# ulrikisdahl/MuZero-Breakout

Measured on AMD Instinct MI355X. Metric: env-steps/sec (whole node) at N_envs×N_sims; visit-count match vs CPU ref, higher is better.
Workload: dtype bf16

## Files before the change

### muzero-breakout_amd/csrc/towerp.hip

```cpp
#include "common.h"
#include "tree_dev.h"
#include "elt.h"

namespace {

constexpr int TP_STAGE = 2;

namespace tp {
constexpr int E = 16;
constexpr int P = 20;
constexpr int ROWS = E * P;
constexpr int C = 256;
constexpr int ROWB = C * 2;
constexpr int IMG = ROWS * ROWB;
constexpr int PIX = E * ROWB;
constexpr int NT = 256;
constexpr int CT = 4;
constexpr int TNS = 72;
constexpr int CTB = TNS * 1024;
MZ_DEV int off(int row, int chunk) { return row * ROWB + ((chunk ^ (row & 15)) << 4); }
MZ_DEV uint32_t relu_pk(uint32_t u) {
  uint32_t r;
  asm("v_pk_max_i16 %0, %1, 0" : "=v"(r) : "v"(u));
  return r;
}
}

#ifdef TOWERP_STAMPS
constexpr int PST_N = 192, PST_WG = 256;
__device__ unsigned long long mz_towerp_stamps[PST_WG * 4][PST_N];
MZ_DEV void pstamp(int k, bool real = false) {
  if ((threadIdx.x & 63) == 0 && blockIdx.x < PST_WG && k < PST_N)
    mz_towerp_stamps[blockIdx.x * 4 + (threadIdx.x >> 6)][k] = real ? __builtin_amdgcn_s_memrealtime() : __builtin_amdgcn_s_memtime();
}
#define PSTAMP(k) pstamp(k)
#else
#define PSTAMP(k) \
  do {            \
  } while (0)
#endif

struct TPW {
  __amdgpu_buffer_rsrc_t rs;
  MZ_DEV uint4 ld(int ct, int step, int lane) const {
    return __builtin_bit_cast(uint4, __builtin_amdgcn_raw_buffer_load_b128(rs, lane * 16, ct * tp::CTB + step * 1024, 0));
  }
};
MZ_DEV TPW tpw(const void* pack, int ct0) {
  const uint4* p = reinterpret_cast<const uint4*>(pack) + (size_t)ct0 * tp::TNS * 64;
  return TPW{__builtin_amdgcn_make_buffer_rsrc(const_cast<uint4*>(p), 0, 0x7fffffff, 0x00020000)};
}

MZ_DEV TPW tpw1(const void* pack, int ct0) {
  const uint4* p = reinterpret_cast<const uint4*>(pack) + (size_t)ct0 * 8 * 64;
  return TPW{__builtin_amdgcn_make_buffer_rsrc(const_cast<uint4*>(p), 0, 0x7fffffff, 0x00020000)};
}

MZ_DEV void tp_preload(uint4 (&bq)[2][3][2], const TPW& w, int lane) {
#pragma unroll
  for (int cc = 0; cc < 2; ++cc)
#pragma unroll
    for (int d = 0; d < 3; ++d)
#pragma unroll
      for (int ct = 0; ct < 2; ++ct) bq[cc][d][ct] = w.ld(ct, 24 * d + cc, lane);
}

template <int EL, int DYI>
__device__ __forceinline__ void tp_dy(const uint8_t* __restrict__ lds, int lb, int q, int n, const TPW& cur,
                                      const TPW& nxt, uint4 (&bq)[2][3][2], f32x4 (&acc)[tp::P][2],
                                      typename Elt<EL>::v8 (&fa)[5], typename Elt<EL>::v8 (&fb)[5], int lane) {
  typedef typename Elt<EL>::v8 V8;
  constexpr int DY = DYI - 1;
  constexpr int YLO = DY < 0 ? 0 : DY, YHI = DY > 0 ? 3 : 3 + DY, NY = YHI - YLO + 1;
  constexpr int NYLO = DYI == 0 ? 0 : (DYI == 1 ? 1 : 0);
#pragma unroll 1
  for (int cp = 0; cp < 4; ++cp) {
#pragma unroll
    for (int cc = 0; cc < 2; ++cc) {
      const int c = 2 * cp + cc, s = 8 * DYI + c;
      const bool wrap = cc == 1 && cp == 3;
      const int cn = wrap ? 0 : c + 1;
      const int xc = lb + (((4 * c + q) ^ n) << 4), xn = lb + (((4 * cn + q) ^ n) << 4);
      const int ynext = wrap ? NYLO : YLO;
      int st = s + 2;
      __amdgpu_buffer_rsrc_t rs = cur.rs;
      if (DYI == 2) {
        rs = st >= 24 ? nxt.rs : cur.rs;
        st = st >= 24 ? st - 24 : st;
      }
#pragma unroll
      for (int yi = 0; yi < NY; ++yi) {
        const int yp = YLO + yi;
        const int nb = yi + 1 < NY ? xc + 5 * (yp + 1) * tp::PIX : xn + 5 * ynext * tp::PIX;
        const bool last = yi == NY - 1;
        auto row = [&](const V8(&f)[5], V8(&fn)[5]) {
          V8 w[3][2];
#pragma unroll
          for (int d = 0; d < 3; ++d)
#pragma unroll
            for (int ct = 0; ct < 2; ++ct) w[d][ct] = __builtin_bit_cast(V8, bq[cc][d][ct]);
#pragma unroll
          for (int xp = 0; xp < 5; ++xp)
#pragma unroll
            for (int ct = 0; ct < 2; ++ct)
              acc[(yp - DY) * 5 + xp][ct] = Elt<EL>::mfma(w[1][ct], f[xp], acc[(yp - DY) * 5 + xp][ct]);
#pragma unroll
          for (int xp = 0; xp < 5; ++xp) fn[xp] = *reinterpret_cast<const V8*>(lds + nb + xp * tp::PIX);
#pragma unroll
          for (int xp = 0; xp < 4; ++xp)
#pragma unroll
            for (int ct = 0; ct < 2; ++ct)
              acc[(yp - DY) * 5 + xp + 1][ct] = Elt<EL>::mfma(w[0][ct], f[xp], acc[(yp - DY) * 5 + xp + 1][ct]);
#pragma unroll
          for (int xp = 1; xp < 5; ++xp)
#pragma unroll
            for (int ct = 0; ct < 2; ++ct)
              acc[(yp - DY) * 5 + xp - 1][ct] = Elt<EL>::mfma(w[2][ct], f[xp], acc[(yp - DY) * 5 + xp - 1][ct]);
          if (last) {
#pragma unroll
            for (int ct = 0; ct < 2; ++ct)
#pragma unroll
              for (int d = 0; d < 3; ++d)
                bq[cc][d][ct] = __builtin_bit_cast(
                    uint4, __builtin_amdgcn_raw_buffer_load_b128(rs, lane * 16, ct * tp::CTB + (24 * d + st) * 1024, 0));
          }
          __builtin_amdgcn_sched_group_barrier(0x008, 8, 0);
#pragma unroll
          for (int j = 0; j < 5; ++j) {
            __builtin_amdgcn_sched_group_barrier(0x008, 1, 0);
            __builtin_amdgcn_sched_group_barrier(0x100, 1, 0);
          }
          __builtin_amdgcn_sched_group_barrier(0x008, 13, 0);
          if (last) __builtin_amdgcn_sched_group_barrier(0x020, 6, 0);
          __builtin_amdgcn_sched_barrier(0);
        };
        if (((cc * NY + yi) & 1) == 0)
          row(fa, fb);
        else
          row(fb, fa);
      }
    }
  }
}

struct TPArgs {
  const bf16_t* in;
  long long in_env_stride;
  const int32_t* slot;
  long long in_slot_stride;
  bf16_t* out;
  const bf16_t* wf;
  const float* bias;
  int nblocks;
  int B;
  mzba_tower_ext x;
  TreeArgs tree;
  int tree_on, tree_sim;
  float tree_gamma;
  const float* tree_r;
};

template <int EL, int MODE>
MZ_DEV void tp_init1(f32x4 (&acc)[2], const float4 (&bias)[2], int chb, const uint2 (&res)[2],
                     const float* __restrict__ actb, int act, int A, int q, int p) {
#pragma unroll
  for (int ct = 0; ct < 2; ++ct) {
    const int ch = chb + 16 * ct + 4 * q;
    const float4 b4 = bias[ct];
    f32x4 v = {b4.x, b4.y, b4.z, b4.w};
    if (MODE == 1) {
      const uint2 r = res[ct];
      v[0] += Elt<EL>::lo(r.x); v[1] += Elt<EL>::hi(r.x);
      v[2] += Elt<EL>::lo(r.y); v[3] += Elt<EL>::hi(r.y);
    } else if (MODE == 2) {
      const float4 t = *reinterpret_cast<const float4*>(actb + ((size_t)p * A + act) * tp::C + ch);
      v[0] += t.x; v[1] += t.y; v[2] += t.z; v[3] += t.w;
    }
    acc[ct] = v;
  }
}
template <int EL, int MODE>
MZ_DEV void tp_init(f32x4 (&acc)[tp::P][2], const float4 (&bias)[2], int chb, const uint2 (&res)[tp::P][2],
                    const float* __restrict__ actb, int act, int A, int q) {
#pragma unroll
  for (int p = 0; p < tp::P; ++p) tp_init1<EL, MODE>(acc[p], bias, chb, res[p], actb, act, A, q, p);
}
MZ_DEV void tp_pin(f32x4 (&acc)[tp::P][2]) {
#pragma unroll
  for (int p = 0; p < tp::P; ++p)
#pragma unroll
    for (int ct = 0; ct < 2; ++ct) asm volatile("" : "+a"(acc[p][ct]));
}

MZ_DEV void tp_bias(float4 (&b)[2], const float* __restrict__ bias, int chb, int q) {
#pragma unroll
  for (int ct = 0; ct < 2; ++ct) b[ct] = *reinterpret_cast<const float4*>(bias + chb + 16 * ct + 4 * q);
}

template <int EL>
MZ_DEV void tp_k3(const uint8_t* __restrict__ lds, int lb, int q, int n, const TPW& cur, const TPW& nxt,
                  uint4 (&bq)[2][3][2], typename Elt<EL>::v8 (&fa)[5], typename Elt<EL>::v8 (&fb)[5],
                  f32x4 (&acc)[tp::P][2], int lane) {
  tp_dy<EL, 0>(lds, lb, q, n, cur, nxt, bq, acc, fa, fb, lane);
  tp_dy<EL, 1>(lds, lb, q, n, cur, nxt, bq, acc, fa, fb, lane);
  tp_dy<EL, 2>(lds, lb, q, n, cur, nxt, bq, acc, fa, fb, lane);
}

template <int EL>
MZ_DEV void tp_k1(const uint8_t* __restrict__ lds, int lb, int q, int n, const TPW& w, f32x4 (&acc)[tp::P][2],
                  int lane) {
  typedef typename Elt<EL>::v8 V8;
  uint4 wq[8][2];
#pragma unroll
  for (int c = 0; c < 8; ++c)
#pragma unroll
    for (int ct = 0; ct < 2; ++ct)
      wq[c][ct] = __builtin_bit_cast(uint4, __builtin_amdgcn_raw_buffer_load_b128(w.rs, lane * 16, ct * 8192 + c * 1024, 0));
  V8 fa[5], fb[5];
  auto rd = [&](int k, V8(&f)[5]) {
    const int xc = lb + (((4 * (k >> 2) + q) ^ n) << 4), yp = k & 3;
#pragma unroll
    for (int xp = 0; xp < 5; ++xp) f[xp] = *reinterpret_cast<const V8*>(lds + xc + (5 * yp + xp) * tp::PIX);
  };
  rd(0, fa);
#pragma unroll
  for (int k = 0; k < 32; ++k) {
    auto step = [&](const V8(&f)[5], V8(&fn)[5]) {
      const int c = k >> 2, yp = k & 3;
      if (k + 1 < 32) rd(k + 1, fn);
#pragma unroll
      for (int ct = 0; ct < 2; ++ct)
#pragma unroll
        for (int xp = 0; xp < 5; ++xp)
          acc[5 * yp + xp][ct] = Elt<EL>::mfma(__builtin_bit_cast(V8, wq[c][ct]), f[xp], acc[5 * yp + xp][ct]);
      if (k + 1 < 32) {
#pragma unroll
        for (int j = 0; j < 5; ++j) {
          __builtin_amdgcn_sched_group_barrier(0x008, 1, 0);
          __builtin_amdgcn_sched_group_barrier(0x100, 1, 0);
        }
        __builtin_amdgcn_sched_group_barrier(0x008, 5, 0);
      }
      __builtin_amdgcn_sched_barrier(0);
    };
    if (k & 1)
      step(fb, fa);
    else
      step(fa, fb);
  }
}

template <int EL>
MZ_DEV uint2 tp_pack(const f32x4& a) {
  return make_uint2(tp::relu_pk(Elt<EL>::pack2(a[0], a[1])), tp::relu_pk(Elt<EL>::pack2(a[2], a[3])));
}
MZ_DEV int tp_cofs(int ch, int n) { return n * tp::ROWB + (((ch >> 3) ^ n) << 4) + ((ch & 7) << 1); }

template <int EL>
MZ_DEV void tp_first_frags(const uint8_t* __restrict__ lds, int lb, int q, int n, typename Elt<EL>::v8 (&fa)[5]) {
  const int x0 = lb + ((q ^ n) << 4);
#pragma unroll
  for (int xp = 0; xp < 5; ++xp) fa[xp] = *reinterpret_cast<const typename Elt<EL>::v8*>(lds + x0 + xp * tp::PIX);
}

template <int EL, int MODE, bool SAVE>
__device__ __forceinline__ void tp_conv(uint8_t* __restrict__ lds, const uint4* w, const TPW& wn,
                                        const float* __restrict__ bias, float4 (&bc)[2], const float* __restrict__ nbias,
                                        uint2 (&res)[2][tp::P][2],
                                        const float* __restrict__ actb, int act, int A, uint4 (&bq)[2][3][2], int lane,
                                        int wave, int ci) {
  const int q = lane >> 4, n = lane & 15;
  const int lb = n * tp::ROWB;
  const int ct0 = tp::CT * wave;
  const TPW w0 = tpw(w, ct0), w1 = tpw(w, ct0 + 2);
  PSTAMP(2 + 5 * ci);
  typename Elt<EL>::v8 fa[5], fb[5];
  tp_first_frags<EL>(lds, lb, q, n, fa);
  uint2 out0[tp::P][2];
  f32x4 acc[tp::P][2];
  tp_init<EL, MODE>(acc, bc, 64 * wave, res[0], actb, act, A, q);
  tp_pin(acc);
  float4 b1[2];
  tp_bias(b1, bias, 64 * wave + 32, q);
  tp_k3<EL>(lds, lb, q, n, w0, w1, bq, fa, fb, acc, lane);
  PSTAMP(3 + 5 * ci);
#pragma unroll
  for (int p = 0; p < tp::P; ++p) {
#pragma unroll
    for (int ct = 0; ct < 2; ++ct) out0[p][ct] = tp_pack<EL>(acc[p][ct]);
    tp_init1<EL, MODE>(acc[p], b1, 64 * wave + 32, res[1][p], actb, act, A, q, p);
    __builtin_amdgcn_sched_barrier(0);
  }
  tp_pin(acc);
  tp_bias(bc, nbias, 64 * wave, q);
  tp_k3<EL>(lds, lb, q, n, w1, wn, bq, fa, fb, acc, lane);
  PSTAMP(4 + 5 * ci);
  __syncthreads();
  PSTAMP(5 + 5 * ci);
  int cofs[tp::CT];
#pragma unroll
  for (int ct = 0; ct < tp::CT; ++ct) cofs[ct] = tp_cofs(64 * wave + 16 * ct + 4 * q, n);
#pragma unroll
  for (int p = 0; p < tp::P; ++p) {
#pragma unroll
    for (int ct = 0; ct < tp::CT; ++ct) {
      uint2* ptr = reinterpret_cast<uint2*>(lds + p * tp::PIX + cofs[ct]);
      if (SAVE) res[ct >> 1][p][ct & 1] = *ptr;
      *ptr = ct < 2 ? out0[p][ct] : tp_pack<EL>(acc[p][ct - 2]);
    }
    __builtin_amdgcn_sched_barrier(0);
  }
  __syncthreads();
  PSTAMP(6 + 5 * ci);
}

constexpr int TPH_PART = 0, TPH_LG = 2048, TPH_DEC = 2560, TPH_TAB = 2688;
template <int EL, int NH, int C0, int C1>
MZ_DEV void tp_heads(const TPArgs& a, uint8_t* __restrict__ lds, const int (&hc0)[2], const int (&kind)[2], int env0,
                     int nenv, int tid) {
  constexpr int NU0 = 20 * C0 / 32 / 4, NU1 = NH > 1 ? 20 * C1 / 32 / 4 : 0, NU = NU0 + NU1;
  static_assert(NU <= 40, "head weight batch");
  const int nh = NH;
  const int lane = tid & 63, wave = tid >> 6, q = lane >> 4, el = lane & 15;
  typedef typename Elt<EL>::v8 V8;
  f32x4 hacc[2] = {{0.f, 0.f, 0.f, 0.f}, {0.f, 0.f, 0.f, 0.f}};
  V8 bv[NU];
#pragma unroll
  for (int u = 0; u < NU; ++u) {
    const int hd = u < NU0 ? 0 : 1, K = 20 * (hd ? C1 : C0), s = wave + 4 * (hd ? u - NU0 : u);
    bv[u] = *reinterpret_cast<const V8*>(reinterpret_cast<const bf16_t*>(a.x.lw[hd]) + (size_t)el * K + s * 32 + q * 8);
  }
#pragma unroll
  for (int u = 0; u < NU; ++u) {
    const int hd = u < NU0 ? 0 : 1, C = hd ? C1 : C0, s = wave + 4 * (hd ? u - NU0 : u);
    const int k = s * 32 + q * 8;
    const int pos = k / C, c = hc0[hd] + (k - pos * C);
    const V8 av = *reinterpret_cast<const V8*>(lds + tp::off(pos * tp::E + el, c >> 3));
    hacc[hd] = Elt<EL>::mfma(av, bv[u], hacc[hd]);
  }
  __syncthreads();
  float* sc = reinterpret_cast<float*>(lds);
  float* part = sc + TPH_PART;
  float* lg = sc + TPH_LG;
  float* dec = sc + TPH_DEC;
#pragma unroll
  for (int hd = 0; hd < 2; ++hd)
    if (hd < nh)
#pragma unroll
      for (int i = 0; i < 4; ++i) part[((hd * 4 + wave) * 16 + 4 * q + i) * 16 + el] = hacc[hd][i];
  __syncthreads();
  for (int hd = 0; hd < nh; ++hd) {
    const int e = tid >> 4, o = tid & 15;
    float v = 0.f;
#pragma unroll
    for (int w = 0; w < 4; ++w) v = v + part[((hd * 4 + w) * 16 + e) * 16 + o];
    if (o < a.x.lO[hd]) lg[(hd * 16 + e) * 16 + o] = v + a.x.lb[hd][o];
  }
  __syncthreads();
  if (tid < 16 * nh) {
    const int hd = tid >> 4, e = tid & 15, b = env0 + e;
    if (e < nenv) {
      const int O = a.x.lO[hd];
      float l[16];
      for (int o = 0; o < O; ++o) {
        l[o] = lg[(hd * 16 + e) * 16 + o];
        if (a.x.logits[hd]) a.x.logits[hd][(size_t)b * O + o] = l[o];
      }
      if (kind[hd] == 0) {
        float m = l[0];
        for (int o = 1; o < O; ++o) m = fmaxf(m, l[o]);
        float ex[16], sum = 0.f;
        for (int o = 0; o < O; ++o) { ex[o] = expf(l[o] - m); sum = sum + ex[o]; }
        for (int o = 0; o < O; ++o) {
          const float p = ex[o] / sum;
          a.x.dec[hd][(size_t)b * O + o] = p;
          if (o < 4) dec[(hd * 16 + e) * 4 + o] = p;
        }
      } else {
        const float d = decode_support(l, O, a.x.smin, a.x.smax);
        a.x.dec[hd][b] = d;
        dec[(hd * 16 + e) * 4] = d;
      }
    }
  }
}

template <int EL>
MZ_DEV void tp_scale(const TPArgs& a, const uint8_t* __restrict__ lds, int env0, int nenv, int tid) {
  const int e = tid >> 4, t = tid & 15;
  uint32_t mn2 = 0xffffffffu, mx2 = 0u;
#pragma unroll 8
  for (int u = 0; u < 40; ++u) {
    const int i = u * 16 + t, p = i >> 5, c = i & 31;
    const uint4 v = *reinterpret_cast<const uint4*>(lds + tp::off(p * tp::E + e, c));
    const uint32_t w4[4] = {v.x, v.y, v.z, v.w};
#pragma unroll
    for (int j = 0; j < 4; ++j) {
      asm("v_pk_min_u16 %0, %1, %2" : "=v"(mn2) : "v"(mn2), "v"(w4[j]));
      asm("v_pk_max_u16 %0, %1, %2" : "=v"(mx2) : "v"(mx2), "v"(w4[j]));
    }
  }
  const uint32_t mnh = min(mn2 & 0xffffu, mn2 >> 16), mxh = max(mx2 & 0xffffu, mx2 >> 16);
  float mn = Elt<EL>::lo(mnh), mx = Elt<EL>::lo(mxh);
  for (int o = 8; o > 0; o >>= 1) { mn = fminf(mn, __shfl_xor(mn, o)); mx = fmaxf(mx, __shfl_xor(mx, o)); }
  if (e >= nenv) return;
  const float den = (mx - mn) + 1e-8f;
  const double rden = 1.0 / (double)den;
  auto dv = [&](float x) { return (float)((double)(x - mn) * rden); };
  const int b = env0 + e;
  bf16_t* o1 = a.out ? a.out + (size_t)b * 20 * tp::C : nullptr;
  bf16_t* o2 = a.x.pool ? reinterpret_cast<bf16_t*>(a.x.pool) + (size_t)b * a.x.pool_env_stride +
                              (size_t)a.x.pool_slot * 20 * tp::C
                        : nullptr;
#pragma unroll 4
  for (int u = 0; u < 40; ++u) {
    const int i = u * 16 + t, p = i >> 5, c = i & 31;
    const uint4 v = *reinterpret_cast<const uint4*>(lds + tp::off(p * tp::E + e, c));
    float f[8];
    unpack8<EL>(v, f);
    const uint4 r = make_uint4(pack_bf16x2(dv(f[0]), dv(f[1])), pack_bf16x2(dv(f[2]), dv(f[3])),
                               pack_bf16x2(dv(f[4]), dv(f[5])), pack_bf16x2(dv(f[6]), dv(f[7])));
    if (o1) *reinterpret_cast<uint4*>(o1 + p * tp::C + c * 8) = r;
    if (o2) *reinterpret_cast<uint4*>(o2 + p * tp::C + c * 8) = r;
  }
}

template <int EL>
__global__ __launch_bounds__(tp::NT, 1) void towerp_kernel(TPArgs a) {
  __shared__ __attribute__((aligned(16))) uint8_t lds[tp::IMG];
  const int tid = threadIdx.x, lane = tid & 63;
  const int wave = __builtin_amdgcn_readfirstlane(tid >> 6);
  const int q = lane >> 4, n = lane & 15, lb = n * tp::ROWB;
  const int env0 = blockIdx.x * tp::E;
  const int nenv = min(tp::E, a.B - env0);
  const uint4* wf = reinterpret_cast<const uint4*>(a.wf);
  constexpr size_t WCONV = (size_t)16 * tp::TNS * 64;
  const bool pro = a.x.w0 != nullptr;
  const int ct0 = tp::CT * wave;
  PSTAMP(0);
#ifdef TOWERP_STAMPS
  pstamp(PST_N - 3, true);
#endif
  uint4 bq[2][3][2];
  tp_preload(bq, tpw(pro ? a.x.w0 : a.wf, ct0), lane);
  const int act = pro ? a.x.act[env0 + (n < nenv ? n : 0)] : 0;
  constexpr int SB = 4 / TP_STAGE;
#pragma unroll
  for (int h = 0; h < TP_STAGE; ++h) {
    uint4 v[10 * SB];
#pragma unroll
    for (int bb = 0; bb < SB; ++bb) {
      const int e = 4 * wave + SB * h + bb;
      const bool ok = e < nenv;
      const int b = env0 + (ok ? e : 0);
      const long long eo = (long long)b * a.in_env_stride + (a.slot ? (long long)a.slot[b] * a.in_slot_stride : 0);
#pragma unroll
      for (int u = 0; u < 10; ++u) {
        v[bb * 10 + u] = Elt<EL>::from_bf16(*reinterpret_cast<const uint4*>(a.in + eo + (long long)(u * 64 + lane) * 8));
        if (!ok) v[bb * 10 + u] = make_uint4(0, 0, 0, 0);
      }
    }
#pragma unroll
    for (int bb = 0; bb < SB; ++bb) {
      const int e = 4 * wave + SB * h + bb;
#pragma unroll
      for (int u = 0; u < 10; ++u) {
        const int cj = u * 64 + lane;
        *reinterpret_cast<uint4*>(lds + tp::off((cj >> 5) * tp::E + e, cj & 31)) = v[bb * 10 + u];
      }
    }
  }
  __syncthreads();
  PSTAMP(1);
  uint2 res[2][tp::P][2];
  const int nconv = 2 * a.nblocks;
  const TPW after = a.x.epilogue == 2 ? tpw(a.x.we3, 2 * wave) : tpw(wf, ct0);
  float4 bc[2];
  tp_bias(bc, pro ? a.x.b0 : a.bias, 64 * wave, q);
  if (pro)
    tp_conv<EL, 2, false>(lds, reinterpret_cast<const uint4*>(a.x.w0), tpw(wf, ct0), a.x.b0, bc, a.bias, res, a.x.act_bias,
                      act, a.x.A, bq, lane, wave, 0);
  const int ci0 = pro ? 1 : 0;
  for (int blk = 0; blk < a.nblocks; ++blk) {
    const int k1 = 2 * blk, k2 = k1 + 1;
    const TPW w3 = k2 + 1 < nconv ? tpw(wf + (k2 + 1) * WCONV, ct0) : after;
    tp_conv<EL, 0, true>(lds, wf + k1 * WCONV, tpw(wf + k2 * WCONV, ct0), a.bias + k1 * tp::C, bc, a.bias + k2 * tp::C, res,
                     nullptr, 0, 0, bq, lane, wave, ci0 + k1);
    tp_conv<EL, 1, false>(lds, wf + k2 * WCONV, w3, a.bias + k2 * tp::C, bc, a.bias + (k2 + 1 < nconv ? k2 + 1 : k2) * tp::C,
                      res, nullptr, 0, 0, bq, lane, wave, ci0 + k2);
  }
  if (a.x.epilogue == 1) {
    uint2 out0[tp::P][2];
    {
      f32x4 acc[tp::P][2];
      float4 b4[2];
      tp_bias(b4, a.x.be1, 64 * wave, q);
      tp_init<EL, 0>(acc, b4, 64 * wave, res[0], nullptr, 0, 0, q);
      tp_pin(acc);
      tp_k1<EL>(lds, lb, q, n, tpw1(a.x.we1, ct0), acc, lane);
#pragma unroll
      for (int p = 0; p < tp::P; ++p)
#pragma unroll
        for (int ct = 0; ct < 2; ++ct) out0[p][ct] = tp_pack<EL>(acc[p][ct]);
    }
    f32x4 acc[tp::P][2];
    float4 b4[2];
    tp_bias(b4, a.x.be1, 64 * wave + 32, q);
    tp_init<EL, 0>(acc, b4, 64 * wave + 32, res[0], nullptr, 0, 0, q);
    tp_pin(acc);
    tp_k1<EL>(lds, lb, q, n, tpw1(a.x.we1, ct0 + 2), acc, lane);
    PSTAMP(160);
    __syncthreads();
    tp_scale<EL>(a, lds, env0, nenv, tid);
    __syncthreads();
    PSTAMP(161);
#pragma unroll
    for (int p = 0; p < tp::P; ++p)
#pragma unroll
      for (int ct = 0; ct < tp::CT; ++ct)
        *reinterpret_cast<uint2*>(lds + p * tp::PIX + tp_cofs(64 * wave + 16 * ct + 4 * q, n)) =
            ct < 2 ? out0[p][ct] : tp_pack<EL>(acc[p][ct - 2]);
    __syncthreads();
    const int hc0[2] = {0, 0}, kind[2] = {1, 0};
    PSTAMP(162);
    tp_heads<EL, 1, tp::C, 0>(a, lds, hc0, kind, env0, nenv, tid);
    PSTAMP(163);
#ifdef TOWERP_STAMPS
    pstamp(PST_N - 2, true);
    pstamp(PST_N - 1);
#endif
    return;
  }
  if (a.x.epilogue == 2) {
    uint2 pol[tp::P][2];
    {
      f32x4 acc[tp::P][2];
      typename Elt<EL>::v8 fa[5], fb[5];
      tp_first_frags<EL>(lds, lb, q, n, fa);
      float4 b4[2];
      tp_bias(b4, a.x.be3, 32 * wave, q);
      tp_init<EL, 0>(acc, b4, 32 * wave, res[0], nullptr, 0, 0, q);
      tp_pin(acc);
      const TPW wp = tpw(a.x.we3, 2 * wave);
      tp_k3<EL>(lds, lb, q, n, wp, wp, bq, fa, fb, acc, lane);
      PSTAMP(160);
#pragma unroll
      for (int p = 0; p < tp::P; ++p)
#pragma unroll
        for (int ct = 0; ct < 2; ++ct) pol[p][ct] = tp_pack<EL>(acc[p][ct]);
    }
    f32x4 acc[tp::P][2];
    float4 b4[2];
    tp_bias(b4, a.x.be1, 32 * wave, q);
    tp_init<EL, 0>(acc, b4, 32 * wave, res[0], nullptr, 0, 0, q);
    tp_pin(acc);
    tp_k1<EL>(lds, lb, q, n, tpw1(a.x.we1, 2 * wave), acc, lane);
    PSTAMP(161);
    __syncthreads();
#pragma unroll
    for (int p = 0; p < tp::P; ++p)
#pragma unroll
      for (int ct = 0; ct < 2; ++ct) {
        *reinterpret_cast<uint2*>(lds + p * tp::PIX + tp_cofs(32 * wave + 16 * ct + 4 * q, n)) = pol[p][ct];
        *reinterpret_cast<uint2*>(lds + p * tp::PIX + tp_cofs(128 + 32 * wave + 16 * ct + 4 * q, n)) = tp_pack<EL>(acc[p][ct]);
      }
    __syncthreads();
    const int ntab = a.tree.S + 1;
    const bool tab_lds = a.tree_on && ntab <= tp::NT;
    float tsq = 0.f, tct = 0.f;
    if (tab_lds && tid < ntab) { tsq = a.tree.sqrt_tab[tid]; tct = a.tree.c_tab[tid]; }
    const int hc0[2] = {0, 128}, kind[2] = {0, 1};
    PSTAMP(162);
    tp_heads<EL, 2, 128, 128>(a, lds, hc0, kind, env0, nenv, tid);
    PSTAMP(163);
    if (a.tree_on) {
      float* sc = reinterpret_cast<float*>(lds);
      float* tab = sc + TPH_TAB;
      if (tab_lds && tid < ntab) { tab[tid] = tsq; tab[ntab + tid] = tct; }
      __syncthreads();
      const float* dec = sc + TPH_DEC;
      if (tid < nenv) {
        const int b = env0 + tid;
        tree_backup_env(a.tree, a.tree_sim, b, a.tree_r[b], dec[(16 + tid) * 4], dec + tid * 4, a.tree_gamma);
        if (a.tree_sim + 1 < a.tree.S)
          tree_select_env(a.tree, a.tree_sim + 1, b, tab_lds ? tab : nullptr, tab_lds ? tab + ntab : nullptr);
      }
    }
    PSTAMP(164);
#ifdef TOWERP_STAMPS
    pstamp(PST_N - 2, true);
    pstamp(PST_N - 1);
#endif
    return;
  }
#pragma unroll
  for (int bb = 0; bb < 4; ++bb) {
    const int e = 4 * wave + bb;
    if (e < nenv) {
#pragma unroll
      for (int u = 0; u < 10; ++u) {
        const int cj = u * 64 + lane;
        *reinterpret_cast<uint4*>(a.out + (long long)(env0 + e) * tp::P * tp::C + (long long)cj * 8) =
            Elt<EL>::to_bf16(*reinterpret_cast<const uint4*>(lds + tp::off((cj >> 5) * tp::E + e, cj & 31)));
      }
    }
  }
#ifdef TOWERP_STAMPS
  pstamp(PST_N - 2, true);
  pstamp(PST_N - 1);
#endif
}

}

extern "C" {

#ifdef TOWERP_STAMPS
int mzba_towerp_stamps_read(unsigned long long* host, int nrows) {
  return (int)hipMemcpyFromSymbol(host, HIP_SYMBOL(mz_towerp_stamps), sizeof(unsigned long long) * PST_N * nrows);
}
#endif

int mzba_towerp_fused(const void* in, long long in_env_stride, const int32_t* slot, long long in_slot_stride,
                      void* out, const void* wf16, const float* bias, int nblocks, int B, const mzba_tower_ext* ext,
                      hipStream_t stream) {
  MZ_CHECK_ARG(B > 0 && nblocks >= 1 && in && wf16 && bias && ext, -1);
  const mzba_tower_ext& x = *ext;
  MZ_CHECK_ARG((x.elem == 0 || x.elem == 1) && x.epilogue >= 0 && x.epilogue <= 2, -2);
  MZ_CHECK_ARG(!x.w0 || (x.b0 && x.act_bias && x.act && x.A > 0), -3);
  MZ_CHECK_ARG(x.epilogue != 0 || out, -3);
  MZ_CHECK_ARG(x.epilogue != 1 || ((out || x.pool) && x.we1 && x.be1 && x.lw[0] && x.lb[0] && x.dec[0] && x.lO[0] > 1 &&
                                   x.lO[0] <= 16), -3);
  MZ_CHECK_ARG(x.epilogue != 2 || (x.we3 && x.be3 && x.we1 && x.be1 && x.lw[0] && x.lw[1] && x.lb[0] && x.lb[1] &&
                                   x.dec[0] && x.dec[1] && x.lO[0] >= 1 && x.lO[0] <= 16 && x.lO[1] > 1 &&
                                   x.lO[1] <= 16), -3);
  TPArgs a{(const bf16_t*)in, in_env_stride, slot, in_slot_stride, (bf16_t*)out, (const bf16_t*)wf16, bias, nblocks, B,
           x, TreeArgs{}, 0, 0, 0.f, nullptr};
  if (x.tree) {
    const mzba_tree_step& t = *x.tree;
    MZ_CHECK_ARG(x.epilogue == 2 && tree_ok_puct(&t) && t.B == B && t.sim >= 0 && t.sim < t.S && t.r, -3);
    a.tree = tree_args(&t);
    a.tree_on = 1;
    a.tree_sim = t.sim;
    a.tree_gamma = t.gamma;
    a.tree_r = t.r;
  }
  if (x.elem == 1)
    hipLaunchKernelGGL(towerp_kernel<1>, dim3((B + tp::E - 1) / tp::E), dim3(tp::NT), 0, stream, a);
  else
    hipLaunchKernelGGL(towerp_kernel<0>, dim3((B + tp::E - 1) / tp::E), dim3(tp::NT), 0, stream, a);
  MZ_LAUNCH_CHECK();
  return 0;
}

int mzba_towerp(const void* in, long long in_env_stride, const int32_t* slot, long long in_slot_stride, void* out,
                const void* wf16, const float* bias, int nblocks, int B, hipStream_t stream) {
  mzba_tower_ext x{};
  return mzba_towerp_fused(in, in_env_stride, slot, in_slot_stride, out, wf16, bias, nblocks, B, &x, stream);
}

}
```

Measured before the change: 32220.

## Remap MFMA output channels so epilogue LDS stores become 16-byte writes

Measured after the change: 32490 (median of 6 runs). No clear change (+0.8%).

```diff
diff --git a/muzero-breakout_amd/csrc/towerp.hip b/muzero-breakout_amd/csrc/towerp.hip
--- a/muzero-breakout_amd/csrc/towerp.hip
+++ b/muzero-breakout_amd/csrc/towerp.hip
@@ -19,6 +19,24 @@
 constexpr int TNS = 72;
 constexpr int CTB = TNS * 1024;
 MZ_DEV int off(int row, int chunk) { return row * ROWB + ((chunk ^ (row & 15)) << 4); }
+
+constexpr int row_ch(int t, int m) { return 8 * (m >> 2) + 4 * t + (m & 3); }
+constexpr int wofs(int stride, int t, int lane) {
+  return (((lane & 15) >> 3)) * stride + (16 * (lane >> 4) + 8 * (((lane & 15) >> 2) & 1) + (lane & 3)) * 16 + 64 * t;
+}
+constexpr int pack_ofs(int stride, int ch, int kq) { return (ch >> 4) * stride + (16 * kq + (ch & 15)) * 16; }
+constexpr bool row_map_ok(int stride) {
+  for (int lane = 0; lane < 64; ++lane)
+    for (int t = 0; t < 2; ++t) {
+      if (wofs(stride, t, lane) != pack_ofs(stride, row_ch(t, lane & 15), lane >> 4)) return false;
+      for (int i = 0; i < 4; ++i)
+        if (row_ch(t, 4 * (lane >> 4) + i) != 8 * (lane >> 4) + 4 * t + i) return false;
+      if ((8 * (lane >> 4) * 2) % 16 != 0) return false;
+    }
+  return true;
+}
+static_assert(row_map_ok(CTB), "row map, 3x3 packs");
+static_assert(row_map_ok(8192), "row map, 1x1 packs");
 MZ_DEV uint32_t relu_pk(uint32_t u) {
   uint32_t r;
   asm("v_pk_max_i16 %0, %1, 0" : "=v"(r) : "v"(u));
@@ -42,8 +60,8 @@
 
 struct TPW {
   __amdgpu_buffer_rsrc_t rs;
-  MZ_DEV uint4 ld(int ct, int step, int lane) const {
-    return __builtin_bit_cast(uint4, __builtin_amdgcn_raw_buffer_load_b128(rs, lane * 16, ct * tp::CTB + step * 1024, 0));
+  MZ_DEV uint4 ld(int t, int step, int wo) const {
+    return __builtin_bit_cast(uint4, __builtin_amdgcn_raw_buffer_load_b128(rs, wo + 64 * t, step * 1024, 0));
   }
 };
 MZ_DEV TPW tpw(const void* pack, int ct0) {
@@ -56,19 +74,19 @@
   return TPW{__builtin_amdgcn_make_buffer_rsrc(const_cast<uint4*>(p), 0, 0x7fffffff, 0x00020000)};
 }
 
-MZ_DEV void tp_preload(uint4 (&bq)[2][3][2], const TPW& w, int lane) {
+MZ_DEV void tp_preload(uint4 (&bq)[2][3][2], const TPW& w, int wo) {
 #pragma unroll
   for (int cc = 0; cc < 2; ++cc)
 #pragma unroll
     for (int d = 0; d < 3; ++d)
 #pragma unroll
-      for (int ct = 0; ct < 2; ++ct) bq[cc][d][ct] = w.ld(ct, 24 * d + cc, lane);
+      for (int ct = 0; ct < 2; ++ct) bq[cc][d][ct] = w.ld(ct, 24 * d + cc, wo);
 }
 
 template <int EL, int DYI>
 __device__ __forceinline__ void tp_dy(const uint8_t* __restrict__ lds, int lb, int q, int n, const TPW& cur,
                                       const TPW& nxt, uint4 (&bq)[2][3][2], f32x4 (&acc)[tp::P][2],
-                                      typename Elt<EL>::v8 (&fa)[5], typename Elt<EL>::v8 (&fb)[5], int lane) {
+                                      typename Elt<EL>::v8 (&fa)[5], typename Elt<EL>::v8 (&fb)[5], int wo) {
   typedef typename Elt<EL>::v8 V8;
   constexpr int DY = DYI - 1;
   constexpr int YLO = DY < 0 ? 0 : DY, YHI = DY > 0 ? 3 : 3 + DY, NY = YHI - YLO + 1;
@@ -118,11 +136,13 @@
               acc[(yp - DY) * 5 + xp - 1][ct] = Elt<EL>::mfma(w[2][ct], f[xp], acc[(yp - DY) * 5 + xp - 1][ct]);
           if (last) {
 #pragma unroll
-            for (int ct = 0; ct < 2; ++ct)
-#pragma unroll
-              for (int d = 0; d < 3; ++d)
+            for (int dd = 0; dd < 3; ++dd) {
+              const int d = dd == 0 ? 1 : (dd == 1 ? 0 : 2);
+#pragma unroll
+              for (int ct = 0; ct < 2; ++ct)
                 bq[cc][d][ct] = __builtin_bit_cast(
-                    uint4, __builtin_amdgcn_raw_buffer_load_b128(rs, lane * 16, ct * tp::CTB + (24 * d + st) * 1024, 0));
+                    uint4, __builtin_amdgcn_raw_buffer_load_b128(rs, wo + 64 * ct, (24 * d + st) * 1024, 0));
+            }
           }
           __builtin_amdgcn_sched_group_barrier(0x008, 8, 0);
 #pragma unroll
@@ -130,8 +150,15 @@
             __builtin_amdgcn_sched_group_barrier(0x008, 1, 0);
             __builtin_amdgcn_sched_group_barrier(0x100, 1, 0);
           }
-          __builtin_amdgcn_sched_group_barrier(0x008, 13, 0);
-          if (last) __builtin_amdgcn_sched_group_barrier(0x020, 6, 0);
+          if (last) {
+            __builtin_amdgcn_sched_group_barrier(0x020, 2, 0);
+            __builtin_amdgcn_sched_group_barrier(0x008, 5, 0);
+            __builtin_amdgcn_sched_group_barrier(0x020, 2, 0);
+            __builtin_amdgcn_sched_group_barrier(0x008, 8, 0);
+            __builtin_amdgcn_sched_group_barrier(0x020, 2, 0);
+          } else {
+            __builtin_amdgcn_sched_group_barrier(0x008, 13, 0);
+          }
           __builtin_amdgcn_sched_barrier(0);
         };
         if (((cc * NY + yi) & 1) == 0)
@@ -161,15 +188,15 @@
 };
 
 template <int EL, int MODE>
-MZ_DEV void tp_init1(f32x4 (&acc)[2], const float4 (&bias)[2], int chb, const uint2 (&res)[2],
+MZ_DEV void tp_init1(f32x4 (&acc)[2], const float4 (&bias)[2], int chb, const uint4& res,
                      const float* __restrict__ actb, int act, int A, int q, int p) {
 #pragma unroll
   for (int ct = 0; ct < 2; ++ct) {
-    const int ch = chb + 16 * ct + 4 * q;
+    const int ch = chb + 8 * q + 4 * ct;
     const float4 b4 = bias[ct];
     f32x4 v = {b4.x, b4.y, b4.z, b4.w};
     if (MODE == 1) {
-      const uint2 r = res[ct];
+      const uint2 r = ct ? make_uint2(res.z, res.w) : make_uint2(res.x, res.y);
       v[0] += Elt<EL>::lo(r.x); v[1] += Elt<EL>::hi(r.x);
       v[2] += Elt<EL>::lo(r.y); v[3] += Elt<EL>::hi(r.y);
     } else if (MODE == 2) {
@@ -180,7 +207,7 @@
   }
 }
 template <int EL, int MODE>
-MZ_DEV void tp_init(f32x4 (&acc)[tp::P][2], const float4 (&bias)[2], int chb, const uint2 (&res)[tp::P][2],
+MZ_DEV void tp_init(f32x4 (&acc)[tp::P][2], const float4 (&bias)[2], int chb, const uint4 (&res)[tp::P],
                     const float* __restrict__ actb, int act, int A, int q) {
 #pragma unroll
   for (int p = 0; p < tp::P; ++p) tp_init1<EL, MODE>(acc[p], bias, chb, res[p], actb, act, A, q, p);
@@ -194,28 +221,27 @@
 
 MZ_DEV void tp_bias(float4 (&b)[2], const float* __restrict__ bias, int chb, int q) {
 #pragma unroll
-  for (int ct = 0; ct < 2; ++ct) b[ct] = *reinterpret_cast<const float4*>(bias + chb + 16 * ct + 4 * q);
+  for (int ct = 0; ct < 2; ++ct) b[ct] = *reinterpret_cast<const float4*>(bias + chb + 8 * q + 4 * ct);
 }
 
 template <int EL>
 MZ_DEV void tp_k3(const uint8_t* __restrict__ lds, int lb, int q, int n, const TPW& cur, const TPW& nxt,
                   uint4 (&bq)[2][3][2], typename Elt<EL>::v8 (&fa)[5], typename Elt<EL>::v8 (&fb)[5],
-                  f32x4 (&acc)[tp::P][2], int lane) {
-  tp_dy<EL, 0>(lds, lb, q, n, cur, nxt, bq, acc, fa, fb, lane);
-  tp_dy<EL, 1>(lds, lb, q, n, cur, nxt, bq, acc, fa, fb, lane);
-  tp_dy<EL, 2>(lds, lb, q, n, cur, nxt, bq, acc, fa, fb, lane);
+                  f32x4 (&acc)[tp::P][2], int wo) {
+  tp_dy<EL, 0>(lds, lb, q, n, cur, nxt, bq, acc, fa, fb, wo);
+  tp_dy<EL, 1>(lds, lb, q, n, cur, nxt, bq, acc, fa, fb, wo);
+  tp_dy<EL, 2>(lds, lb, q, n, cur, nxt, bq, acc, fa, fb, wo);
 }
 
 template <int EL>
 MZ_DEV void tp_k1(const uint8_t* __restrict__ lds, int lb, int q, int n, const TPW& w, f32x4 (&acc)[tp::P][2],
-                  int lane) {
+                  int wo1) {
   typedef typename Elt<EL>::v8 V8;
   uint4 wq[8][2];
 #pragma unroll
   for (int c = 0; c < 8; ++c)
 #pragma unroll
-    for (int ct = 0; ct < 2; ++ct)
-      wq[c][ct] = __builtin_bit_cast(uint4, __builtin_amdgcn_raw_buffer_load_b128(w.rs, lane * 16, ct * 8192 + c * 1024, 0));
+    for (int ct = 0; ct < 2; ++ct) wq[c][ct] = w.ld(ct, c, wo1);
   V8 fa[5], fb[5];
   auto rd = [&](int k, V8(&f)[5]) {
     const int xc = lb + (((4 * (k >> 2) + q) ^ n) << 4), yp = k & 3;
@@ -251,10 +277,11 @@
 }
 
 template <int EL>
-MZ_DEV uint2 tp_pack(const f32x4& a) {
-  return make_uint2(tp::relu_pk(Elt<EL>::pack2(a[0], a[1])), tp::relu_pk(Elt<EL>::pack2(a[2], a[3])));
-}
-MZ_DEV int tp_cofs(int ch, int n) { return n * tp::ROWB + (((ch >> 3) ^ n) << 4) + ((ch & 7) << 1); }
+MZ_DEV uint4 tp_pack(const f32x4 (&a)[2]) {
+  return make_uint4(tp::relu_pk(Elt<EL>::pack2(a[0][0], a[0][1])), tp::relu_pk(Elt<EL>::pack2(a[0][2], a[0][3])),
+                    tp::relu_pk(Elt<EL>::pack2(a[1][0], a[1][1])), tp::relu_pk(Elt<EL>::pack2(a[1][2], a[1][3])));
+}
+MZ_DEV int tp_cofs(int chb, int q, int n) { return n * tp::ROWB + ((((chb >> 3) + q) ^ n) << 4); }
 
 template <int EL>
 MZ_DEV void tp_first_frags(const uint8_t* __restrict__ lds, int lb, int q, int n, typename Elt<EL>::v8 (&fa)[5]) {
@@ -266,9 +293,9 @@
 template <int EL, int MODE, bool SAVE>
 __device__ __forceinline__ void tp_conv(uint8_t* __restrict__ lds, const uint4* w, const TPW& wn,
                                         const float* __restrict__ bias, float4 (&bc)[2], const float* __restrict__ nbias,
-                                        uint2 (&res)[2][tp::P][2],
+                                        uint4 (&res)[2][tp::P],
                                         const float* __restrict__ actb, int act, int A, uint4 (&bq)[2][3][2], int lane,
-                                        int wave, int ci) {
+                                        int wo, int wave, int ci) {
   const int q = lane >> 4, n = lane & 15;
   const int lb = n * tp::ROWB;
   const int ct0 = tp::CT * wave;
@@ -276,37 +303,36 @@
   PSTAMP(2 + 5 * ci);
   typename Elt<EL>::v8 fa[5], fb[5];
   tp_first_frags<EL>(lds, lb, q, n, fa);
-  uint2 out0[tp::P][2];
+  uint4 out0[tp::P];
   f32x4 acc[tp::P][2];
   tp_init<EL, MODE>(acc, bc, 64 * wave, res[0], actb, act, A, q);
   tp_pin(acc);
   float4 b1[2];
   tp_bias(b1, bias, 64 * wave + 32, q);
-  tp_k3<EL>(lds, lb, q, n, w0, w1, bq, fa, fb, acc, lane);
+  tp_k3<EL>(lds, lb, q, n, w0, w1, bq, fa, fb, acc, wo);
   PSTAMP(3 + 5 * ci);
 #pragma unroll
   for (int p = 0; p < tp::P; ++p) {
-#pragma unroll
-    for (int ct = 0; ct < 2; ++ct) out0[p][ct] = tp_pack<EL>(acc[p][ct]);
+    out0[p] = tp_pack<EL>(acc[p]);
     tp_init1<EL, MODE>(acc[p], b1, 64 * wave + 32, res[1][p], actb, act, A, q, p);
     __builtin_amdgcn_sched_barrier(0);
   }
   tp_pin(acc);
   tp_bias(bc, nbias, 64 * wave, q);
-  tp_k3<EL>(lds, lb, q, n, w1, wn, bq, fa, fb, acc, lane);
+  tp_k3<EL>(lds, lb, q, n, w1, wn, bq, fa, fb, acc, wo);
   PSTAMP(4 + 5 * ci);
   __syncthreads();
   PSTAMP(5 + 5 * ci);
-  int cofs[tp::CT];
-#pragma unroll
-  for (int ct = 0; ct < tp::CT; ++ct) cofs[ct] = tp_cofs(64 * wave + 16 * ct + 4 * q, n);
+  int cofs[2];
+#pragma unroll
+  for (int ps = 0; ps < 2; ++ps) cofs[ps] = tp_cofs(64 * wave + 32 * ps, q, n);
 #pragma unroll
   for (int p = 0; p < tp::P; ++p) {
 #pragma unroll
-    for (int ct = 0; ct < tp::CT; ++ct) {
-      uint2* ptr = reinterpret_cast<uint2*>(lds + p * tp::PIX + cofs[ct]);
-      if (SAVE) res[ct >> 1][p][ct & 1] = *ptr;
-      *ptr = ct < 2 ? out0[p][ct] : tp_pack<EL>(acc[p][ct - 2]);
+    for (int ps = 0; ps < 2; ++ps) {
+      uint4* ptr = reinterpret_cast<uint4*>(lds + p * tp::PIX + cofs[ps]);
+      if (SAVE) res[ps][p] = *ptr;
+      *ptr = ps == 0 ? out0[p] : tp_pack<EL>(acc[p]);
     }
     __builtin_amdgcn_sched_barrier(0);
   }
@@ -441,8 +467,9 @@
 #ifdef TOWERP_STAMPS
   pstamp(PST_N - 3, true);
 #endif
+  const int wo = tp::wofs(tp::CTB, 0, lane), wo1 = tp::wofs(8192, 0, lane);
   uint4 bq[2][3][2];
-  tp_preload(bq, tpw(pro ? a.x.w0 : a.wf, ct0), lane);
+  tp_preload(bq, tpw(pro ? a.x.w0 : a.wf, ct0), wo);
   const int act = pro ? a.x.act[env0 + (n < nenv ? n : 0)] : 0;
   constexpr int SB = 4 / TP_STAGE;
 #pragma unroll
@@ -472,54 +499,51 @@
   }
   __syncthreads();
   PSTAMP(1);
-  uint2 res[2][tp::P][2];
+  uint4 res[2][tp::P];
   const int nconv = 2 * a.nblocks;
   const TPW after = a.x.epilogue == 2 ? tpw(a.x.we3, 2 * wave) : tpw(wf, ct0);
   float4 bc[2];
   tp_bias(bc, pro ? a.x.b0 : a.bias, 64 * wave, q);
   if (pro)
     tp_conv<EL, 2, false>(lds, reinterpret_cast<const uint4*>(a.x.w0), tpw(wf, ct0), a.x.b0, bc, a.bias, res, a.x.act_bias,
-                      act, a.x.A, bq, lane, wave, 0);
+                      act, a.x.A, bq, lane, wo, wave, 0);
   const int ci0 = pro ? 1 : 0;
   for (int blk = 0; blk < a.nblocks; ++blk) {
     const int k1 = 2 * blk, k2 = k1 + 1;
     const TPW w3 = k2 + 1 < nconv ? tpw(wf + (k2 + 1) * WCONV, ct0) : after;
     tp_conv<EL, 0, true>(lds, wf + k1 * WCONV, tpw(wf + k2 * WCONV, ct0), a.bias + k1 * tp::C, bc, a.bias + k2 * tp::C, res,
-                     nullptr, 0, 0, bq, lane, wave, ci0 + k1);
+                     nullptr, 0, 0, bq, lane, wo, wave, ci0 + k1);
     tp_conv<EL, 1, false>(lds, wf + k2 * WCONV, w3, a.bias + k2 * tp::C, bc, a.bias + (k2 + 1 < nconv ? k2 + 1 : k2) * tp::C,
-                      res, nullptr, 0, 0, bq, lane, wave, ci0 + k2);
+                      res, nullptr, 0, 0, bq, lane, wo, wave, ci0 + k2);
   }
   if (a.x.epilogue == 1) {
-    uint2 out0[tp::P][2];
+    uint4 out0[tp::P];
     {
       f32x4 acc[tp::P][2];
       float4 b4[2];
       tp_bias(b4, a.x.be1, 64 * wave, q);
       tp_init<EL, 0>(acc, b4, 64 * wave, res[0], nullptr, 0, 0, q);
       tp_pin(acc);
-      tp_k1<EL>(lds, lb, q, n, tpw1(a.x.we1, ct0), acc, lane);
-#pragma unroll
-      for (int p = 0; p < tp::P; ++p)
-#pragma unroll
-        for (int ct = 0; ct < 2; ++ct) out0[p][ct] = tp_pack<EL>(acc[p][ct]);
+      tp_k1<EL>(lds, lb, q, n, tpw1(a.x.we1, ct0), acc, wo1);
+#pragma unroll
+      for (int p = 0; p < tp::P; ++p) out0[p] = tp_pack<EL>(acc[p]);
     }
     f32x4 acc[tp::P][2];
     float4 b4[2];
     tp_bias(b4, a.x.be1, 64 * wave + 32, q);
     tp_init<EL, 0>(acc, b4, 64 * wave + 32, res[0], nullptr, 0, 0, q);
     tp_pin(acc);
-    tp_k1<EL>(lds, lb, q, n, tpw1(a.x.we1, ct0 + 2), acc, lane);
+    tp_k1<EL>(lds, lb, q, n, tpw1(a.x.we1, ct0 + 2), acc, wo1);
     PSTAMP(160);
     __syncthreads();
     tp_scale<EL>(a, lds, env0, nenv, tid);
     __syncthreads();
     PSTAMP(161);
 #pragma unroll
-    for (int p = 0; p < tp::P; ++p)
-#pragma unroll
-      for (int ct = 0; ct < tp::CT; ++ct)
-        *reinterpret_cast<uint2*>(lds + p * tp::PIX + tp_cofs(64 * wave + 16 * ct + 4 * q, n)) =
-            ct < 2 ? out0[p][ct] : tp_pack<EL>(acc[p][ct - 2]);
+    for (int p = 0; p < tp::P; ++p) {
+      *reinterpret_cast<uint4*>(lds + p * tp::PIX + tp_cofs(64 * wave, q, n)) = out0[p];
+      *reinterpret_cast<uint4*>(lds + p * tp::PIX + tp_cofs(64 * wave + 32, q, n)) = tp_pack<EL>(acc[p]);
+    }
     __syncthreads();
     const int hc0[2] = {0, 0}, kind[2] = {1, 0};
     PSTAMP(162);
@@ -532,7 +556,7 @@
     return;
   }
   if (a.x.epilogue == 2) {
-    uint2 pol[tp::P][2];
+    uint4 pol[tp::P];
     {
       f32x4 acc[tp::P][2];
       typename Elt<EL>::v8 fa[5], fb[5];
@@ -542,28 +566,24 @@
       tp_init<EL, 0>(acc, b4, 32 * wave, res[0], nullptr, 0, 0, q);
       tp_pin(acc);
       const TPW wp = tpw(a.x.we3, 2 * wave);
-      tp_k3<EL>(lds, lb, q, n, wp, wp, bq, fa, fb, acc, lane);
+      tp_k3<EL>(lds, lb, q, n, wp, wp, bq, fa, fb, acc, wo);
       PSTAMP(160);
 #pragma unroll
-      for (int p = 0; p < tp::P; ++p)
-#pragma unroll
-        for (int ct = 0; ct < 2; ++ct) pol[p][ct] = tp_pack<EL>(acc[p][ct]);
+      for (int p = 0; p < tp::P; ++p) pol[p] = tp_pack<EL>(acc[p]);
     }
     f32x4 acc[tp::P][2];
     float4 b4[2];
     tp_bias(b4, a.x.be1, 32 * wave, q);
     tp_init<EL, 0>(acc, b4, 32 * wave, res[0], nullptr, 0, 0, q);
     tp_pin(acc);
-    tp_k1<EL>(lds, lb, q, n, tpw1(a.x.we1, 2 * wave), acc, lane);
+    tp_k1<EL>(lds, lb, q, n, tpw1(a.x.we1, 2 * wave), acc, wo1);
     PSTAMP(161);
     __syncthreads();
 #pragma unroll
-    for (int p = 0; p < tp::P; ++p)
-#pragma unroll
-      for (int ct = 0; ct < 2; ++ct) {
-        *reinterpret_cast<uint2*>(lds + p * tp::PIX + tp_cofs(32 * wave + 16 * ct + 4 * q, n)) = pol[p][ct];
-        *reinterpret_cast<uint2*>(lds + p * tp::PIX + tp_cofs(128 + 32 * wave + 16 * ct + 4 * q, n)) = tp_pack<EL>(acc[p][ct]);
-      }
+    for (int p = 0; p < tp::P; ++p) {
+      *reinterpret_cast<uint4*>(lds + p * tp::PIX + tp_cofs(32 * wave, q, n)) = pol[p];
+      *reinterpret_cast<uint4*>(lds + p * tp::PIX + tp_cofs(128 + 32 * wave, q, n)) = tp_pack<EL>(acc[p]);
+    }
     __syncthreads();
     const int ntab = a.tree.S + 1;
     const bool tab_lds = a.tree_on && ntab <= tp::NT;
```
